# ideafisher/ssUnet-GAN

Hardware: AMD Instinct MI355X
Metric: train images/sec (512^2 tiles) (higher is better)
Workload: dtype f32; 1 GPU; UNet_R_SS_v2 generator + SRGAN-style discriminator, one G+D step (train_seg_gan.py:182-233), 16 x 3x512x512 tiles per GPU, fp32, Adam lr 2e-5; global_batch=16, tile=512, parallelism=dp1, dead_d_param_grads_of_g_step=computed

## Files before the change

### ssunet-gan_amd/csrc/conv_wgrad.hip

```cpp
#include "common.h"
#include "conv_thin.h"
#include "conv_wgrad_args.h"
#include <stdlib.h>

namespace {

constexpr int BKP = 16;

template <int BM, int BN, int WAVES_M, int WAVES_N>
__global__ __launch_bounds__(256) void wgrad_kernel(const WgArgs a) {
  constexpr int WTM = BM / WAVES_M, WTN = BN / WAVES_N;
  constexpr int MI = WTM / 32, NI = WTN / 32;
  constexpr int LDA = BM + 4, LDB = BN + 4;
  constexpr int AQ = BM / 4, BQ = BN / 4;
  constexpr int A_LD = BKP * AQ / 256, B_LD = (BKP * BQ + 255) / 256;
  constexpr int A_PSTEP = 256 / AQ, B_PSTEP = 256 / BQ;
  static_assert(A_LD >= 1, "tile");

  __shared__ __attribute__((aligned(16))) float lds[2 * BKP * (LDA + LDB)];
  float* As = lds;
  float* Bs = lds + 2 * BKP * LDA;

  const int tid = threadIdx.x, lane = tid & 63, wave = tid >> 6;
  const int wm = wave / WAVES_N, wn = wave % WAVES_N;
// ... 91 lines not shown
  }

  float* slab = a.ws + (size_t)blockIdx.z * a.M * a.Cout;
#pragma unroll
  for (int i = 0; i < MI; ++i)
#pragma unroll
    for (int j = 0; j < NI; ++j) {
      const int co = n0 + wn * WTN + j * 32 + l31;
#pragma unroll
      for (int r = 0; r < 16; ++r) {
        const int row = m0 + wm * WTM + i * 32 + (r & 3) + 8 * (r >> 2) + 4 * half;
        if (row < a.M && co < a.Cout) slab[(size_t)row * a.Cout + co] = acc[i][j][r];
      }
    }
}

struct RedArgs {
  const float* ws; float* dw; int splits, M, Cout, Cin, Cin_real, KH, KW, ntaps;
  int ky[SSG_MAX_TAPS], kx[SSG_MAX_TAPS];
};

template <int ZL>
__global__ __launch_bounds__(32 * ZL) void wgrad_reduce_kernel(const RedArgs a) {
  __shared__ float red[ZL][32];
  const int el = threadIdx.x & 31, zl = threadIdx.x >> 5;
  const long long idx = (long long)blockIdx.x * 32 + el;
  const long long tot = (long long)a.M * a.Cout;
  float s = 0.f;
  if (idx < tot) {
    int z = zl;
    for (; z + 3 * ZL < a.splits; z += 4 * ZL) {
      const float v0 = a.ws[(size_t)z * tot + idx], v1 = a.ws[(size_t)(z + ZL) * tot + idx];
      const float v2 = a.ws[(size_t)(z + 2 * ZL) * tot + idx], v3 = a.ws[(size_t)(z + 3 * ZL) * tot + idx];
      s += v0; s += v1; s += v2; s += v3;
    }
    for (; z < a.splits; z += ZL) s += a.ws[(size_t)z * tot + idx];
  }
  red[zl][el] = s;
  __syncthreads();
  if (zl != 0 || idx >= tot) return;
  float v = 0.f;
#pragma unroll
  for (int k = 0; k < ZL; ++k) v += red[k][el];
  const int row = (int)(idx / a.Cout), co = (int)(idx - (long long)row * a.Cout);
  const int t = row / a.Cin, c = row - t * a.Cin;
  if (c >= a.Cin_real) return;
  a.dw[(((size_t)co * a.Cin_real + c) * a.KH + a.ky[t]) * a.KW + a.kx[t]] = v;
}

struct Plan { int variant, mt, nt, splits, steps_per_split, halo; };

int wgrad4_kind(const ssg_wgrad_desc* d) {
  static const int on = [] { const char* e = getenv("SSG_WGRAD4"); return e ? atoi(e) : 1; }();
  return on ? ssg_wgrad4_kind(d) : 0;
}

bool wgrad_uses_dma(int variant) {
  static const int use_dma = [] { const char* e = getenv("SSG_WGRAD_DMA"); return e ? atoi(e) : 1; }();
  return use_dma && variant <= 1;
}

bool wgrad_uses_halo(const ssg_wgrad_desc* d, int variant) {
  static const int on = [] { const char* e = getenv("SSG_WGRAD_HALO"); return e ? atoi(e) : 1; }();
  return on && variant <= 1 && wgrad_uses_dma(variant) && ssg_wgrad_halo_ok(d, variant);
}

Plan make_plan(const ssg_wgrad_desc* d) {
  Plan p;
  p.halo = 0;
  const int Cin = d->C1 + d->C2;
  const int M = d->ntaps * Cin;
  int bn;
  if (d->Cout > 64) { p.variant = 0; bn = 128; }
  else if (d->Cout > 32) { p.variant = 1; bn = 64; }
  else { p.variant = 2; bn = 32; }
  p.mt = (M + 127) / 128;
  p.nt = (d->Cout + bn - 1) / bn;
  long long steps = ((long long)d->N * d->GH * d->GW + BKP - 1) / BKP;
  if (wgrad_uses_halo(d, p.variant)) {
    p.halo = 1;
    p.mt = Cin / ssg_wgrad_halo_cb(p.variant);
    steps = (long long)d->N * d->GH * ((d->GW + BKP - 1) / BKP);
  }
  if ((d->flags & 1) && ssg_wgrad_k32_ok(d)) {
    p.halo = 2;
    p.mt = Cin / 64; p.nt = d->Cout / 64;
    steps = ssg_wgrad_k32_steps(d);
    const long long tiles = (long long)p.mt * p.nt;
    long long max_rows = 128;
    {
      const long long steps16 = (long long)d->N * d->GH * ((d->GW + BKP - 1) / BKP);
      const long long mtf = Cin / ssg_wgrad_halo_cb(p.variant), ntf = (d->Cout + (p.variant == 0 ? 127 : 63)) / (p.variant == 0 ? 128 : 64);
      long long wantf = 1024 / (mtf * ntf > 0 ? mtf * ntf : 1);
      if (wantf < 1) wantf = 1;
      if (wantf > steps16 / 16) wantf = steps16 / 16 > 0 ? steps16 / 16 : 1;
      if (wantf > 512) wantf = 512;
      const long long chain_px = (steps16 + wantf - 1) / wantf * BKP;
      if (chain_px / 32 < max_rows) max_rows = chain_px / 32;
      if (max_rows < 8) max_rows = 8;
    }
    const long long lo = ssg_wgrad_k32_flush() == 0 ? (steps + max_rows - 1) / max_rows : 1;
    long long hi = steps / 8;
    if (hi < lo) hi = lo;
    long long best = lo; double beff = 0;
    for (long long sp = lo; sp <= hi && sp <= lo + 1024; ++sp) {
      const long long wg = sp * tiles;
      const double eff = (double)wg / (256.0 * ((wg + 255) / 256));
      if (eff > beff + 1e-9) { beff = eff; best = sp; }
      if (eff >= 0.97 && wg >= 256) break;
    }
    p.steps_per_split = (int)((steps + best - 1) / best);
    p.splits = (int)((steps + p.steps_per_split - 1) / p.steps_per_split);
    return p;
  }
  static const int wgs = [] { const char* e = getenv("SSG_WGRAD_WGS"); return e ? atoi(e) : 1024; }();
  long long want = wgs / ((long long)p.mt * p.nt);
  if (want < 1) want = 1;
  long long maxs = steps / 16;
  if (maxs < 1) maxs = 1;
  if (want > maxs) want = maxs;
  if (want > 512) want = 512;
  p.steps_per_split = (int)((steps + want - 1) / want);
  p.splits = (int)((steps + p.steps_per_split - 1) / p.steps_per_split);
  return p;
}

int validate(const ssg_wgrad_desc* d) {
  SSG_REQUIRE(d && d->in1 && d->dout && d->dw_oihw, SSG_EINVAL, "wgrad: null pointer");
  SSG_REQUIRE(d->C1 > 0 && d->C1 % 4 == 0 && d->C2 >= 0 && d->C2 % 4 == 0, SSG_EINVAL, "wgrad: channels must be multiples of 4");
  SSG_REQUIRE(d->C2 == 0 || d->in2, SSG_EINVAL, "wgrad: C2 > 0 needs in2");
  SSG_REQUIRE(d->ld1 % 4 == 0 && d->ld1 >= d->C1 && d->ldd % 4 == 0 && d->ldd >= d->Cout, SSG_EALIGN, "wgrad: strides");
  SSG_REQUIRE(d->C2 == 0 || (d->ld2 % 4 == 0 && d->ld2 >= d->C2), SSG_EALIGN, "wgrad: ld2");
  SSG_REQUIRE(ssg_aligned16(d->in1) && ssg_aligned16(d->in2) && ssg_aligned16(d->dout) && ssg_aligned16(d->ws), SSG_EALIGN, "wgrad: alignment");
  SSG_REQUIRE(d->ntaps >= 1 && d->ntaps <= SSG_MAX_TAPS, SSG_EINVAL, "wgrad: ntaps");
  SSG_REQUIRE(d->Cin_real > 0 && d->Cin_real <= d->C1 + d->C2, SSG_EINVAL, "wgrad: Cin_real");
  for (int t = 0; t < d->ntaps; ++t) {
    SSG_REQUIRE(d->dy[t] >= -2 && d->dy[t] <= 5 && d->dx[t] >= -2 && d->dx[t] <= 5, SSG_EINVAL, "wgrad: tap offset");
    SSG_REQUIRE(d->ky[t] >= 0 && d->ky[t] < d->KH && d->kx[t] >= 0 && d->kx[t] < d->KW, SSG_EINVAL, "wgrad: kernel position");
  }
  SSG_REQUIRE(d->ws_bytes >= ssg_conv2d_wgrad_workspace_bytes(d), SSG_EINVAL, "wgrad: workspace too small");
  return SSG_OK;
}

__global__ __launch_bounds__(256) void pack_weights_kernel(const float* __restrict__ w, int O, int I, int KH, int KW,
                                                           int transpose, int ntaps, unsigned long long kpos_bits,
                                                           int kmode, int Cred_pad, int Kp, int R, float* __restrict__ out,
                                                           const float* __restrict__ sigma) {
  const long long idx = (long long)blockIdx.x * 256 + threadIdx.x;
  if (idx >= (long long)R * Kp) return;
  const int r = (int)(idx / Kp), k = (int)(idx - (long long)r * Kp);
  int t, c;
  if (kmode == 0) {
    const int span = ntaps * 16;
    const int chunk = k / span, rem = k - chunk * span;
    t = rem >> 4; c = chunk * 16 + (rem & 15);
  } else {
    t = k / Cred_pad; c = k - t * Cred_pad;
  }
  const int Cred = transpose ? O : I;
  float v = 0.f;
  if (t < ntaps && c < Cred) {
    const int kb = (int)((kpos_bits >> (6 * t)) & 63ull);
    const int ky = kb & 7, kx = kb >> 3;
    const int o = transpose ? c : r, i = transpose ? r : c;
    v = w[(((size_t)o * I + i) * KH + ky) * KW + kx];
    if (sigma) v *= 1.f / *sigma;
  }
  out[idx] = v;
}

}

extern "C" int64_t ssg_conv2d_wgrad_workspace_bytes(const ssg_wgrad_desc* d) {
  if (!d) return 0;
  if (wgrad4_kind(d)) {
    const int nz = ssg_wgrad4_slices(d, wgrad4_kind(d), nullptr, nullptr, nullptr);
    return (int64_t)nz * d->ntaps * (d->C1 + d->C2) * d->Cout * (int64_t)sizeof(float);
  }
  const Plan p = make_plan(d);
  return (int64_t)p.splits * d->ntaps * (d->C1 + d->C2) * d->Cout * (int64_t)sizeof(float);
}

extern "C" int ssg_conv2d_wgrad_in_affine_ok(const ssg_wgrad_desc* d) {
  if (!d || !d->in1 || !d->dout || wgrad4_kind(d)) return 0;
  if (d->C2 != 0 || (d->in_act != SSG_ACT_NONE && d->in_act != SSG_ACT_RELU && d->in_act != SSG_ACT_LRELU)) return 0;
  return make_plan(d).halo == 2 ? 1 : 0;
}

extern "C" int ssg_conv2d_wgrad_f32(const ssg_wgrad_desc* d, void* stream) {
  int rc = validate(d);
  if (rc != SSG_OK) return rc;
  SSG_REQUIRE(!d->in_scale || (d->in_shift && ssg_conv2d_wgrad_in_affine_ok(d)), SSG_EINVAL,
              "wgrad: in_scale on a descriptor whose kernel has no fused input transform (ssg_conv2d_wgrad_in_affine_ok == 0)");
  Plan p = make_plan(d);
  hipStream_t st = (hipStream_t)stream;
  const int w4 = wgrad4_kind(d);
  WgArgs a;
  a.in1 = d->in1; a.in2 = d->C2 ? d->in2 : d->in1; a.dout = d->dout; a.ws = d->ws;
  a.C1 = d->C1; a.C2 = d->C2; a.ld1 = d->ld1; a.ld2 = d->C2 ? d->ld2 : d->ld1;
  a.N = d->N; a.H = d->H; a.W = d->W; a.Cout = d->Cout; a.ldd = d->ldd; a.GH = d->GH; a.GW = d->GW;
  a.in_sy = d->in_sy; a.in_sx = d->in_sx; a.ntaps = d->ntaps;
  a.tap_bits = 0;
  for (int t = 0; t < d->ntaps; ++t)
    a.tap_bits |= (unsigned long long)(((d->dy[t] + 2) & 7) | (((d->dx[t] + 2) & 7) << 3)) << (6 * t);
  a.in_scale = d->in_scale; a.in_shift = d->in_shift; a.in_act = d->in_act; a.in_slope = d->in_slope;
  a.M = d->ntaps * (d->C1 + d->C2);
  a.Ptot = (long long)d->N * d->GH * d->GW;
  a.steps_per_split = p.steps_per_split;
  if (w4) {
    p.splits = ssg_wgrad4_slices(d, w4, nullptr, nullptr, nullptr);
    rc = ssg_wgrad4_launch(d, w4, st);
    if (rc != SSG_OK) return rc;
  } else {
    dim3 grid((unsigned)p.mt, (unsigned)p.nt, (unsigned)p.splits);
    if (p.halo == 2) {
      rc = ssg_wgrad_k32_launch(a, grid, st);
      if (rc != SSG_OK) return rc;
    } else if (p.halo) {
      rc = ssg_wgrad_halo_launch(a, p.variant, grid, st, (d->flags & 1) != 0);
      if (rc != SSG_OK) return rc;
    } else if (wgrad_uses_dma(p.variant)) {
      rc = ssg_wgrad_dma_launch(a, p.variant, grid, st, (d->flags & 1) != 0);
      if (rc != SSG_OK) return rc;
    } else
    switch (p.variant) {
      case 0: hipLaunchKernelGGL((wgrad_kernel<128, 128, 2, 2>), grid, dim3(256), 0, st, a); break;
      case 1: hipLaunchKernelGGL((wgrad_kernel<128, 64, 2, 2>), grid, dim3(256), 0, st, a); break;
      default: hipLaunchKernelGGL((wgrad_kernel<128, 32, 4, 1>), grid, dim3(256), 0, st, a); break;
    }
    SSG_LAUNCH_CHECK();
  }
  RedArgs r;
  r.ws = d->ws; r.dw = d->dw_oihw; r.splits = p.splits; r.M = a.M; r.Cout = d->Cout; r.Cin = d->C1 + d->C2;
  r.Cin_real = d->Cin_real; r.KH = d->KH; r.KW = d->KW; r.ntaps = d->ntaps;
  for (int t = 0; t < SSG_MAX_TAPS; ++t) { r.ky[t] = t < d->ntaps ? d->ky[t] : 0; r.kx[t] = t < d->ntaps ? d->kx[t] : 0; }
  const long long tot = (long long)a.M * d->Cout;
  if (p.splits >= 256 && tot <= 32 * 1024)
    hipLaunchKernelGGL(wgrad_reduce_kernel<32>, dim3((unsigned)ssg_cdiv(tot, 32)), dim3(1024), 0, st, r);
  else
    hipLaunchKernelGGL(wgrad_reduce_kernel<8>, dim3((unsigned)ssg_cdiv(tot, 32)), dim3(256), 0, st, r);
  SSG_LAUNCH_CHECK();
  return SSG_OK;
}

extern "C" int ssg_pack_weights_scaled_f32(const float* w_oihw, int O, int I, int KH, int KW, int transpose, int ntaps,
                                           const int* ky, const int* kx, int kmode, int Cred_pad, int Kp, const float* sigma, float* out,
                                           void* stream);
extern "C" int ssg_pack_weights_f32(const float* w_oihw, int O, int I, int KH, int KW, int transpose, int ntaps,
                                    const int* ky, const int* kx, int kmode, int Cred_pad, int Kp, float* out,
                                    void* stream) {
  return ssg_pack_weights_scaled_f32(w_oihw, O, I, KH, KW, transpose, ntaps, ky, kx, kmode, Cred_pad, Kp, nullptr, out, stream);
}
extern "C" int ssg_pack_weights_scaled_f32(const float* w_oihw, int O, int I, int KH, int KW, int transpose, int ntaps,
                                           const int* ky, const int* kx, int kmode, int Cred_pad, int Kp, const float* sigma, float* out,
                                           void* stream) {
  SSG_REQUIRE(w_oihw && out && ky && kx, SSG_EINVAL, "pack: null pointer");
  SSG_REQUIRE(ntaps >= 1 && ntaps <= SSG_MAX_TAPS && KH <= 8 && KW <= 8, SSG_EINVAL, "pack: taps");
  SSG_REQUIRE(Kp % 16 == 0 && Cred_pad % 4 == 0, SSG_EINVAL, "pack: Kp/Cred_pad");
  const int Cred = transpose ? O : I;
  SSG_REQUIRE(Cred_pad >= Cred, SSG_EINVAL, "pack: Cred_pad < reduced channels");
  if (kmode == 0) SSG_REQUIRE(Cred_pad % 16 == 0 && Kp == ntaps * Cred_pad, SSG_EINVAL, "pack: kmode 0 shape");
  else SSG_REQUIRE(Kp >= ntaps * Cred_pad, SSG_EINVAL, "pack: kmode 1 Kp");
  unsigned long long bits = 0;
  for (int t = 0; t < ntaps; ++t) {
    SSG_REQUIRE(ky[t] >= 0 && ky[t] < KH && kx[t] >= 0 && kx[t] < KW, SSG_EINVAL, "pack: kernel position");
    bits |= (unsigned long long)(ky[t] | (kx[t] << 3)) << (6 * t);
  }
  const int R = transpose ? I : O;
  const long long tot = (long long)R * Kp;
  hipLaunchKernelGGL(pack_weights_kernel, dim3((unsigned)ssg_cdiv(tot, 256)), dim3(256), 0, (hipStream_t)stream,
                     w_oihw, O, I, KH, KW, transpose, ntaps, bits, kmode, Cred_pad, Kp, R, out, sigma);
  SSG_LAUNCH_CHECK();
  return SSG_OK;
}

extern "C" int ssg_conv2d_wgrad_kernel_id(const ssg_wgrad_desc* d) {
  if (!d) return SSG_EINVAL;
  if (wgrad4_kind(d)) return 10 + wgrad4_kind(d);
  if (make_plan(d).halo == 2) return 60;
  if (make_plan(d).halo) return ((d->flags & 1) ? 40 : 30) + make_plan(d).variant;
  const int v = make_plan(d).variant;
  return v + (wgrad_uses_dma(v) ? ((d->flags & 1) ? 50 : 20) : 0);
}
```

### ssunet-gan_amd/csrc/conv_wgrad_args.h

```cpp
#pragma once
#include "common.h"

struct WgArgs {
  const float* in1; const float* in2; const float* dout; float* ws;
  int C1, C2, ld1, ld2, N, H, W, Cout, ldd, GH, GW, in_sy, in_sx, ntaps;
  unsigned long long tap_bits;
  int M;
  long long Ptot;
  int steps_per_split;
  int xcd_swizzle;
  const float* in_scale; const float* in_shift; int in_act; float in_slope;
};


int ssg_wgrad_dma_launch(const WgArgs& a, int variant, dim3 grid, hipStream_t st, bool split);

int ssg_wgrad_halo_cb(int variant);
bool ssg_wgrad_halo_ok(const ssg_wgrad_desc* d, int variant);
int ssg_wgrad_halo_launch(const WgArgs& a, int variant, dim3 grid, hipStream_t st, bool split);

bool ssg_wgrad_k32_ok(const ssg_wgrad_desc* d);
long long ssg_wgrad_k32_steps(const ssg_wgrad_desc* d);
int ssg_wgrad_k32_flush();
int ssg_wgrad_k32_launch(const WgArgs& a, dim3 grid, hipStream_t st);
```

### ssunet-gan_amd/csrc/conv_wgrad_k32.hip

```cpp
#include "common.h"
#include "lds_dma.h"
#include "conv_wgrad_args.h"
#include "mfma_split.h"
#include "conv_slow.h"
#include <stdlib.h>

namespace {

typedef unsigned u32x4 __attribute__((ext_vector_type(4)));
typedef short s16x4 __attribute__((ext_vector_type(4)));
typedef short s16x8 __attribute__((ext_vector_type(8)));
typedef __attribute__((address_space(3))) s16x4 lds_s16x4;

constexpr int KP = 32;
constexpr int WPX = 36;
constexpr int XSLOT = WPX * 128;
constexpr int XPLANE = 4 * XSLOT;
constexpr int XIMG = 3 * XPLANE;
constexpr int DSLOT = KP * 128;
constexpr int DPLANE = 2 * DSLOT;
constexpr int DIMG = 3 * DPLANE;
constexpr int CB = 64, BN = 64;
#ifndef SSG_WK32_FLUSH
#define SSG_WK32_FLUSH 0
#endif

__device__ __forceinline__ int sw(int p) { return ((((p >> 1) & 1) | (((p >> 3) & 1) << 1)) << 1); }

template <bool XF>
__global__ __launch_bounds__(512, 1) void wgrad_k32_kernel(const WgArgs a) {
  extern __shared__ __attribute__((aligned(1024))) unsigned char lds[];
  unsigned char* const ximg = lds;
  unsigned char* const dimg = lds + XIMG;

  const int tid = threadIdx.x, lane = tid & 63;
  const int wave = __builtin_amdgcn_readfirstlane(tid >> 6);
  const int wm = wave >> 1, wn = wave & 1;
  const int l15 = lane & 15, g = lane >> 4;
  const int c0 = blockIdx.x * CB, n0 = blockIdx.y * BN;
  const int Cin = a.C1 + a.C2;
  const int XB = (a.GW + KP - 1) / KP;

  const long long total = (long long)a.N * XB * a.GH;
  long long S0 = (long long)blockIdx.z * a.steps_per_split, S1 = S0 + a.steps_per_split;
  if (S1 > total) S1 = total;

  const unsigned OOB = 0xffffffffu;
  const bool first = c0 < a.C1;
  const float* xsrc = first ? a.in1 : a.in2;
  const int xld = first ? a.ld1 : a.ld2;
  const int xc0 = first ? c0 : c0 - a.C1;
  const unsigned npix = (unsigned)a.N * (unsigned)a.H * (unsigned)a.W;
  const auto x_rs = __builtin_amdgcn_make_buffer_rsrc(const_cast<float*>(xsrc), 0, (int)(npix * (unsigned)xld * 4u), 0x00020000);
  const auto d_rs = __builtin_amdgcn_make_buffer_rsrc(const_cast<float*>(a.dout), 0, (int)((unsigned)a.N * (unsigned)a.GH * (unsigned)a.GW * (unsigned)a.ldd * 4u), 0x00020000);

  const int s_px = tid >> 4, s_q = tid & 15;
  const bool has_x2 = tid < 32;
  const int x_dst = s_px * 128 + (((s_q >> 1) ^ sw(s_px)) << 4) + (s_q & 1) * 8;
  const int x_dst2 = (32 + s_px) * 128 + (((s_q >> 1) ^ sw(32 + s_px)) << 4) + (s_q & 1) * 8;
  const int d_dst = x_dst;

  struct RawX { u32x4 a, b; };
  struct RawD { u32x4 a; };
  float* const xtab = (float*)(lds + XIMG + DIMG);
  if constexpr (XF) {
    if (tid < 128) xtab[tid] = tid < 64 ? a.in_scale[c0 + tid] : a.in_shift[c0 + tid - 64];
  }
  auto x_inside = [&](int row, int gx0, int px) -> bool {
    return (unsigned)row < (unsigned)a.H && (unsigned)(gx0 - 1 + px) < (unsigned)a.W;
  };
  auto load_x = [&](int n, int row, int gx0) -> RawX {
    const unsigned rowbase = (unsigned)((n * a.H + row) * a.W + gx0 - 1);
    const unsigned cho = (unsigned)(xc0 + 4 * s_q) * 4u;
    const unsigned vo = x_inside(row, gx0, s_px) ? (rowbase + (unsigned)s_px) * (unsigned)xld * 4u + cho : OOB;
    const unsigned vo2 = (has_x2 && x_inside(row, gx0, 32 + s_px)) ? (rowbase + 32u + (unsigned)s_px) * (unsigned)xld * 4u + cho : OOB;
    RawX r;
    r.a = __builtin_amdgcn_raw_buffer_load_b128(x_rs, vo, 0, 0);
    r.b = __builtin_amdgcn_raw_buffer_load_b128(x_rs, vo2, 0, 0);
    return r;
  };
  auto load_d = [&](int n, int gy, int gx0) -> RawD {
    const int gx = gx0 + s_px;
    const unsigned vo = gx < a.GW ? (unsigned)((n * a.GH + gy) * a.GW + gx) * (unsigned)a.ldd * 4u + (unsigned)(n0 + 4 * s_q) * 4u : OOB;
    RawD r;
    r.a = __builtin_amdgcn_raw_buffer_load_b128(d_rs, vo, 0, 0);
    return r;
  };
  auto put = [&](unsigned char* base, int plane_bytes, f32x4 v) {
    bf16x4 p1, p2, p3;
    split3_4(v, p1, p2, p3);
    *(bf16x4*)base = p1; *(bf16x4*)(base + plane_bytes) = p2; *(bf16x4*)(base + 2 * plane_bytes) = p3;
  };
  auto xform = [&](f32x4 v, bool inside) -> f32x4 {
    if constexpr (XF) {
      v = v * *(const f32x4*)(xtab + 4 * s_q) + *(const f32x4*)(xtab + 64 + 4 * s_q);
#pragma unroll
      for (int e = 0; e < 4; ++e) v[e] = ssg_act(v[e], a.in_act, a.in_slope);
      if (!inside) v = f32x4{0.f, 0.f, 0.f, 0.f};
    }
    return v;
  };
  auto store_x = [&](const RawX& r, int slot, int row, int gx0) {
    put(ximg + slot * XSLOT + x_dst, XPLANE, xform(__builtin_bit_cast(f32x4, r.a), XF ? x_inside(row, gx0, s_px) : true));
    if (has_x2) put(ximg + slot * XSLOT + x_dst2, XPLANE, xform(__builtin_bit_cast(f32x4, r.b), XF ? x_inside(row, gx0, 32 + s_px) : true));
  };
  auto store_d = [&](const RawD& r, int slot) {
    put(dimg + slot * DSLOT + d_dst, DPLANE, __builtin_bit_cast(f32x4, r.a));
  };

  const int q4 = l15 >> 2, pp = l15 & 3;
  int xoff[3][2], doff[2][2];
#pragma unroll
  for (int t = 0; t < 2; ++t) {
#pragma unroll
    for (int dx = 0; dx < 3; ++dx) {
      const int p = dx + 8 * g + q4 + 4 * t;
      xoff[dx][t] = p * 128 + ((((2 * wm + (pp >> 1)) ^ sw(p))) << 4) + (pp & 1) * 8;
    }
    const int p = 8 * g + q4 + 4 * t;
#pragma unroll
    for (int j = 0; j < 2; ++j)
      doff[j][t] = p * 128 + ((((2 * (2 * wn + j) + (pp >> 1)) ^ sw(p))) << 4) + (pp & 1) * 8;
  }

  constexpr int FLUSH = SSG_WK32_FLUSH;
  f32x4 acc[9][2], tot[9][2];
#pragma unroll
  for (int t = 0; t < 9; ++t)
#pragma unroll
    for (int j = 0; j < 2; ++j) { acc[t][j] = f32x4{0.f, 0.f, 0.f, 0.f}; tot[t][j] = f32x4{0.f, 0.f, 0.f, 0.f}; }
  int since = 0;

  auto frag = [&](const unsigned char* base, int o0, int o1) -> bf16x8 {
    const s16x4 lo = __builtin_amdgcn_ds_read_tr16_b64_v4i16((lds_s16x4*)(base + o0));
    const s16x4 hi = __builtin_amdgcn_ds_read_tr16_b64_v4i16((lds_s16x4*)(base + o1));
    const s16x8 v = __builtin_shufflevector(lo, hi, 0, 1, 2, 3, 4, 5, 6, 7);
    return __builtin_bit_cast(bf16x8, v);
  };

  long long S = S0;
  while (S < S1) {
    const int strip = (int)(S / a.GH), ga = (int)(S - (long long)strip * a.GH);
    long long Se = (long long)(strip + 1) * a.GH;
    if (Se > S1) Se = S1;
    const int gb = ga + (int)(Se - S);
    const int n = strip / XB, gx0 = (strip - n * XB) * KP;

    wait_lds_reads();
    __builtin_amdgcn_s_barrier();
    asm volatile("" ::: "memory");
    {
      const RawX r0 = load_x(n, ga - 1, gx0), r1 = load_x(n, ga, gx0), r2 = load_x(n, ga + 1, gx0);
      const RawD r3 = load_d(n, ga, gx0);
      store_x(r0, (ga + 0) & 3, ga - 1, gx0); store_x(r1, (ga + 1) & 3, ga, gx0);
      store_x(r2, (ga + 2) & 3, ga + 1, gx0); store_d(r3, ga & 1);
    }

    for (int gy = ga; gy < gb; ++gy) {
      wait_lds_reads();
      __builtin_amdgcn_s_barrier();
      asm volatile("" ::: "memory");
      const bool more = gy + 1 < gb;
      RawX nx; RawD nd;
#ifndef SSG_WK32_LOAD_MID
#define SSG_WK32_LOAD_MID 0
#endif
#if !SSG_WK32_LOAD_MID
      if (more) { nx = load_x(n, gy + 2, gx0); nd = load_d(n, gy + 1, gx0); }
#endif

      const unsigned char* db = dimg + (gy & 1) * DSLOT;
      bf16x8 df[2][3];
#pragma unroll
      for (int j = 0; j < 2; ++j)
#pragma unroll
        for (int q = 0; q < 3; ++q) df[j][q] = frag(db + q * DPLANE, doff[j][0], doff[j][1]);
#pragma unroll
      for (int dyi = 0; dyi < 3; ++dyi) {
#ifndef SSG_WK32_DYNPRIO
#define SSG_WK32_DYNPRIO 1
#endif
        if (SSG_WK32_DYNPRIO) { if (dyi == 0) __builtin_amdgcn_s_setprio(3); else if (dyi == 1) __builtin_amdgcn_s_setprio(2); else __builtin_amdgcn_s_setprio(1); }
        const unsigned char* xb = ximg + ((gy + dyi) & 3) * XSLOT;
        bf16x8 xf[3][3];
#pragma unroll
        for (int dx = 0; dx < 3; ++dx)
#pragma unroll
          for (int q = 0; q < 3; ++q) xf[dx][q] = frag(xb + q * XPLANE, xoff[dx][0], xoff[dx][1]);
#define SSG_WK_TERM(QD, QX)                                                                       \
  _Pragma("unroll") for (int dx = 0; dx < 3; ++dx)                                                \
  _Pragma("unroll") for (int j = 0; j < 2; ++j)                                                   \
      acc[dyi * 3 + dx][j] = __builtin_amdgcn_mfma_f32_16x16x32_bf16(df[j][QD], xf[dx][QX], acc[dyi * 3 + dx][j], 0, 0, 0);
        SSG_WK_TERM(2, 0) SSG_WK_TERM(1, 1) SSG_WK_TERM(0, 2)
        SSG_WK_TERM(1, 0) SSG_WK_TERM(0, 1)
        SSG_WK_TERM(0, 0)
#undef SSG_WK_TERM
#if SSG_WK32_LOAD_MID
        if (dyi == 0) {
          __builtin_amdgcn_sched_barrier(0);
          if (more) { nx = load_x(n, gy + 2, gx0); nd = load_d(n, gy + 1, gx0); }
          __builtin_amdgcn_sched_barrier(0);
        }
#endif
      }
      if (SSG_WK32_DYNPRIO) __builtin_amdgcn_s_setprio(0);
      if (more) {
        __builtin_amdgcn_sched_barrier(0);
        store_x(nx, (gy + 3) & 3, gy + 2, gx0);
        store_d(nd, (gy + 1) & 1);
      }
      if (FLUSH > 0 && ++since == FLUSH) {
        since = 0;
#pragma unroll
        for (int t = 0; t < 9; ++t)
#pragma unroll
          for (int j = 0; j < 2; ++j) { tot[t][j] += acc[t][j]; acc[t][j] = f32x4{0.f, 0.f, 0.f, 0.f}; }
      }
    }
    S = Se;
  }
#pragma unroll
  for (int t = 0; t < 9; ++t)
#pragma unroll
    for (int j = 0; j < 2; ++j) tot[t][j] += acc[t][j];

  wait_lds_reads();
  {
    bool bad = false;
#pragma unroll
    for (int t = 0; t < 9; ++t)
#pragma unroll
      for (int j = 0; j < 2; ++j)
#pragma unroll
        for (int r = 0; r < 4; ++r) bad |= ssg_nonfinite(tot[t][j][r]);
    if (__builtin_amdgcn_readfirstlane(__syncthreads_or(bad))) {
      const WgArgs& as = *ssg_reload_args<WgArgs>();
#pragma unroll
      for (int t = 0; t < 9; ++t)
#pragma unroll
        for (int j = 0; j < 2; ++j)
          ssg_slow_refill4(tot[t][j], (float*)lds + tid, 512, [&](int r) {
            return ssg_wgrad_slow_value_strips<XF>(as, t, c0 + wm * 16 + l15, n0 + (2 * wn + j) * 16 + 4 * g + r, S0, S1, KP);
          });
    }
  }

  float* slab = a.ws + (size_t)blockIdx.z * a.M * a.Cout;
  const int ci = c0 + wm * 16 + l15;
#pragma unroll
  for (int t = 0; t < 9; ++t)
#pragma unroll
    for (int j = 0; j < 2; ++j)
      *(f32x4*)(slab + ((size_t)t * Cin + ci) * a.Cout + n0 + (2 * wn + j) * 16 + 4 * g) = tot[t][j];
}

}

static int g_wk32_mode = -1;
extern "C" int ssg_wgrad_set_k32_mode(int mode) {
  SSG_REQUIRE(mode == 0 || mode == 1, SSG_EINVAL, "wgrad k32 mode %d", mode);
  g_wk32_mode = mode;
  return SSG_OK;
}

bool ssg_wgrad_k32_ok(const ssg_wgrad_desc* d) {
  if (g_wk32_mode < 0) { const char* e = getenv("SSG_WGRAD_K32"); g_wk32_mode = e ? atoi(e) : 1; }
  if (!g_wk32_mode || !(d->flags & 1)) return false;
  if (d->ntaps != 9 || d->in_sy != 1 || d->in_sx != 1 || d->GH != d->H || d->GW != d->W) return false;
  for (int t = 0; t < 9; ++t)
    if (d->dy[t] != t / 3 - 1 || d->dx[t] != t % 3 - 1) return false;
  if (d->C1 % 64 || d->C2 % 64 || d->Cout % 64 || d->GW < 17) return false;
  if ((d->ld1 & 3) || (d->C2 && (d->ld2 & 3)) || (d->ldd & 3)) return false;
  const unsigned long long xb = (unsigned long long)d->N * d->H * d->W * (unsigned long long)(d->ld1 > d->ld2 ? d->ld1 : d->ld2) * 4ull;
  const unsigned long long db = (unsigned long long)d->N * d->GH * d->GW * (unsigned long long)d->ldd * 4ull;
  return xb <= 0xfffffff0ull && db <= 0xfffffff0ull;
}

int ssg_wgrad_k32_flush() { return SSG_WK32_FLUSH; }

long long ssg_wgrad_k32_steps(const ssg_wgrad_desc* d) { return (long long)d->N * ((d->GW + KP - 1) / KP) * d->GH; }

int ssg_wgrad_k32_launch(const WgArgs& a, dim3 grid, hipStream_t st) {
  constexpr int lds_bytes = XIMG + DIMG;
  static const hipError_t attr = hipFuncSetAttribute((const void*)wgrad_k32_kernel<false>, hipFuncAttributeMaxDynamicSharedMemorySize, lds_bytes);
  static const hipError_t attr_xf = hipFuncSetAttribute((const void*)wgrad_k32_kernel<true>, hipFuncAttributeMaxDynamicSharedMemorySize, lds_bytes + 512);
  if (attr != hipSuccess || attr_xf != hipSuccess) { ssg_set_error("wgrad k32: LDS attribute: %s", hipGetErrorString(attr != hipSuccess ? attr : attr_xf)); return (int)(attr != hipSuccess ? attr : attr_xf); }
  if (a.in_scale) hipLaunchKernelGGL(wgrad_k32_kernel<true>, grid, dim3(512), lds_bytes + 512, st, a);
  else hipLaunchKernelGGL(wgrad_k32_kernel<false>, grid, dim3(512), lds_bytes, st, a);
  SSG_LAUNCH_CHECK();
  return SSG_OK;
}
```

### ssunet-gan_amd/ops.py

```python
import ctypes as C
import math

import torch
import torch.distributed as dist

from . import _lib
from ._lib import ACT_LRELU, ACT_NONE, ACT_RELU, ConvDesc, WgradDesc, call, ptr, stream_ptr

__all__ = ['conv2d', 'batch_norm_act', 'max_pool2x2', 'max_pool2x2_skip', 'max_unpool2x2', 'upsample2x_bilinear', 'upsample2x_nearest',
           'spade_modulate', 'adaptive_avgpool_flat', 'linear', 'seg_loss', 'bce_with_logits_const', 'nan_to_zero_',
           'to_nhwc', 'new_nhwc', 'bump_weight_epoch', 'dwconv2d', 'swish', 'sigmoid', 'gaussian', 'mul', 'global_avgpool',
           'channel_scale', 'spectral_norm_weight', 'conv2d_sn']


def pad4(c):
    return (c + 3) // 4 * 4


def new_nhwc(n, c, h, w, device, ld=None, zero=False):
    ld = pad4(c) if ld is None else ld
    buf = (torch.zeros if zero else torch.empty)(n * h * w * ld, device=device, dtype=torch.float32)
    return torch.empty(0, device=device, dtype=torch.float32).set_(
        buf.untyped_storage(), 0, (n, c, h, w), (h * w * ld, 1, w * ld, ld))

# ... 99 lines not shown
    cache = weight.__dict__.get('_ssg_pack')
    if cache is None or cache[0] != stamp:
        cache = (stamp, {})
        try:
            weight._ssg_pack = cache
        except Exception:
            pass
    key = (transpose, tuple(taps), cred_pad, kmode)
    hit = cache[1].get(key)
    if hit is not None:
        return hit, kp, kmode
    out = torch.empty((rows, kp), device=weight.device, dtype=torch.float32)
    ky = (C.c_int * nt)(*[t[0] for t in taps])
    kx = (C.c_int * nt)(*[t[1] for t in taps])
    call('ssg_pack_weights_f32', ptr(weight), o, i, kh, kw, int(transpose), nt, ky, kx, kmode, cred_pad, kp, ptr(out), stream_ptr())
    cache[1][key] = out
    return out, kp, kmode


def _fill_taps(desc, taps):
    desc.ntaps = len(taps)
    for t, (_, _, dy, dx) in enumerate(taps):
        desc.dy[t] = dy
        desc.dx[t] = dx


PROFILE = None
PROFILE_SHAPES = False
PROFILE_HBM = None
PROFILE_COMM = None
_ROLE = [None]


def _timed_all_reduce(kind, t, group):
    if PROFILE_COMM is None:
        dist.all_reduce(t, op=dist.ReduceOp.SUM, group=group)
        return
    e0 = torch.cuda.Event(enable_timing=True); e1 = torch.cuda.Event(enable_timing=True)
    e0.record(torch.cuda.current_stream())
    dist.all_reduce(t, op=dist.ReduceOp.SUM, group=group)
    e1.record(torch.cuda.current_stream())
    PROFILE_COMM.append((kind, t.numel() * t.element_size(), e0, e1))


class role(object):

    def __init__(self, name):
        self.name = name

    def __enter__(self):
        self.prev = _ROLE[0]; _ROLE[0] = self.name

    def __exit__(self, *a):
        _ROLE[0] = self.prev


class _hbm(object):

    def __init__(self, stage, nbytes):
        self.rec = PROFILE_HBM is not None
        if self.rec:
            self.stage, self.nbytes = stage, float(nbytes)
            self.e0 = torch.cuda.Event(enable_timing=True); self.e1 = torch.cuda.Event(enable_timing=True)

    def __enter__(self):
        if self.rec:
            self.e0.record(torch.cuda.current_stream())

    def __exit__(self, *a):
        if self.rec:
            self.e1.record(torch.cuda.current_stream())
            PROFILE_HBM.append((self.stage, self.nbytes, self.e0, self.e1))


_CONV_LABELS = {0: 'conv_igemm_kernel<128,128>', 1: 'conv_igemm_kernel<256,64>', 2: 'conv_igemm_kernel<256,32>',
                20: 'conv_igemm_dma_kernel<128,128>', 21: 'conv_igemm_dma_kernel<256,64>', 22: 'conv_igemm_dma_kernel<128,64>',
                30: 'conv_igemm_halo_kernel<128,128>', 31: 'conv_igemm_halo_kernel<256,64>', 32: 'conv_igemm_halo_kernel<128,64>',
                33: 'conv_igemm_halo16_kernel<128,128>', 34: 'conv_igemm_halo16_kernel<128,64>',
                10: 'thin_small_cout_kernel',
                12: 'thin4_cin_kernel', 13: 'thin4_cout_kernel', 14: 'tiny4_kernel', 15: 'thin32_cin_kernel', 16: 'conv1x1_k64_kernel'}
_WGRAD_LABELS = {0: 'wgrad_kernel<128,128>', 1: 'wgrad_kernel<128,64>', 2: 'wgrad_kernel<128,32>',
                 20: 'wgrad_dma_kernel<128,128>', 21: 'wgrad_dma_kernel<128,64>',
                 30: 'wgrad_halo_kernel<32,128>', 31: 'wgrad_halo_kernel<64,64>',
                 40: 'wgrad_halo_x3_kernel<32,128>', 41: 'wgrad_halo_x3_kernel<64,64>', 60: 'wgrad_k32_kernel<64,64>',
                 50: 'wgrad_dma_x3_kernel<128,128>', 51: 'wgrad_dma_x3_kernel<128,64>',
                 15: 'wgrad4_kernel<thin_cout>', 16: 'wgrad4_kernel<thin_cin>', 17: 'wgrad_tiny4_kernel', 18: 'wgrad32_cin_kernel'}


class _Timed(object):
    def __init__(self, label, flops, tag=None):
        self.rec = PROFILE is not None
        if self.rec:
            self.label, self.flops, self.tag = label, flops, tag
            self.e0 = torch.cuda.Event(enable_timing=True); self.e1 = torch.cuda.Event(enable_timing=True)

    def __enter__(self):
        if self.rec:
            self.e0.record(torch.cuda.current_stream())

    def __exit__(self, *a):
        if self.rec:
            self.e1.record(torch.cuda.current_stream())
            PROFILE.append((self.label, self.flops, self.e0, self.e1, self.tag))


_DECLINED = object()


def _conv_launch(x1, x2, wpk, kp, kmode, row0, cout, bias, res, act, slope, taps, n, h, w, gh, gw, oh, ow,
                 in_s, out_s, out_oy, out_ox, out, want_bn=False, tag=None, parity_merge=False, in_affine=None, bwd_stats=None):
    d = ConvDesc()
    d.in1 = x1.data_ptr(); d.C1 = pad4(x1.shape[1]); d.ld1 = _ld(x1)
    if x2 is not None:
        d.in2 = x2.data_ptr(); d.C2 = pad4(x2.shape[1]); d.ld2 = _ld(x2)
    else:
        d.in2 = None; d.C2 = 0; d.ld2 = 0
    d.N, d.H, d.W = n, h, w
    d.w = wpk.data_ptr() + row0 * kp * 4; d.Kp = kp; d.kmode = kmode
    d.bias = bias.data_ptr() if bias is not None else None
    if res is not None:
        d.res = res.data_ptr(); d.ldr = _ld(res)
    else:
        d.res = None; d.ldr = 0
    d.out = out.data_ptr(); d.Cout = cout; d.ldo = _ld(out)
    d.GH, d.GW, d.OH, d.OW = gh, gw, oh, ow
    d.in_sy = d.in_sx = in_s
    d.out_sy = d.out_sx = out_s
    d.out_oy, d.out_ox = out_oy, out_ox
    _fill_taps(d, taps)
    d.act = act; d.slope = slope
    d.bnpart = None
    d.ws = None; d.ws_bytes = 0
    d.w_split = None
    d.parity_merge = 1 if parity_merge else 0
    d.in_scale = None; d.in_shift = None; d.in_act = ACT_NONE; d.in_slope = 0.0
    d.bwd_x = None; d.bwd_ldx = 0; d.bwd_scale = None; d.bwd_shift = None; d.bwd_mean = None; d.bwd_act = ACT_NONE; d.bwd_slope = 0.0
    split = None
    if parity_merge and not (MFMA_SPLIT and kmode == 0 and call('ssg_conv2d_split_bn', C.byref(d)) == 64):
        return False
    if MFMA_SPLIT and kmode == 0:
        bn = call('ssg_conv2d_split_bn', C.byref(d))
        if bn:
            split = _split_pack(wpk, row0, cout, kp, 1064 if bn == 2064 else bn)
            d.w_split = split.data_ptr()
    if in_affine is not None:
        d.in_scale = in_affine[0].data_ptr(); d.in_shift = in_affine[1].data_ptr(); d.in_act = int(in_affine[2]); d.in_slope = float(in_affine[3])
        if split is None or not call('ssg_conv2d_in_affine_ok', C.byref(d)):
            return _DECLINED
        bn = call('ssg_conv2d_split_bn', C.byref(d))
    if bwd_stats is not None:
        bx, bst, bact, bslope = bwd_stats
        d.bwd_x = bx.data_ptr(); d.bwd_ldx = _ld(bx); d.bwd_scale = bst[2].data_ptr(); d.bwd_shift = bst[3].data_ptr()
        d.bwd_mean = bst[0].data_ptr(); d.bwd_act = int(bact); d.bwd_slope = float(bslope)
        if split is None or not call('ssg_conv2d_bwd_stats_ok', C.byref(d)):
            return _DECLINED
        want_bn = True
    part = None
    if want_bn and BN_EPILOGUE:
        rows = call('ssg_conv2d_bnpart_rows', C.byref(d))
        if rows > 0:
            part = torch.empty((rows, 2, cout), dtype=torch.float64, device=out.device)
            d.bnpart = part.data_ptr()
    if bwd_stats is not None and part is None:
        return _DECLINED
    ws = None
    if part is None and split is None:
        need = call('ssg_conv2d_workspace_bytes', C.byref(d))
# ... 1210 lines not shown
```

Baseline: 85.63 images/sec.

## Extend k32 weight-gradient kernel to stride-2 3x3 convolutions

Adds a stride-2 variant of the LDS-staged k32 wgrad kernel. Input rows are stored de-interleaved by even and odd column in a five-slot ring, and two input rows are loaded per output row. This routes stride-2 3x3 convs, which previously fell back to the generic or DMA wgrad kernels, onto the faster fused path. The path is gated on having enough tiles to fill the GPU, and it needs more LDS and an extra row load per step.

```diff
diff --git a/ssunet-gan_amd/csrc/conv_wgrad.hip b/ssunet-gan_amd/csrc/conv_wgrad.hip
--- a/ssunet-gan_amd/csrc/conv_wgrad.hip
+++ b/ssunet-gan_amd/csrc/conv_wgrad.hip
@@ -197,13 +197,23 @@
     p.mt = Cin / ssg_wgrad_halo_cb(p.variant);
     steps = (long long)d->N * d->GH * ((d->GW + BKP - 1) / BKP);
   }
-  if ((d->flags & 1) && ssg_wgrad_k32_ok(d)) {
-    p.halo = 2;
+  const bool k32_s2 = (d->flags & 1) && !p.halo && ssg_wgrad_k32_s2_ok(d);
+  if (((d->flags & 1) && ssg_wgrad_k32_ok(d)) || k32_s2) {
+    p.halo = k32_s2 ? 3 : 2;
     p.mt = Cin / 64; p.nt = d->Cout / 64;
     steps = ssg_wgrad_k32_steps(d);
     const long long tiles = (long long)p.mt * p.nt;
     long long max_rows = 128;
-    {
+    if (k32_s2) {
+      const long long steps16 = ((long long)d->N * d->GH * d->GW + BKP - 1) / BKP;
+      long long wantf = 1024 / ((long long)((M + 127) / 128) * ((d->Cout + bn - 1) / bn));
+      if (wantf < 1) wantf = 1;
+      if (wantf > steps16 / 16) wantf = steps16 / 16 > 0 ? steps16 / 16 : 1;
+      if (wantf > 512) wantf = 512;
+      const long long chain_px = (steps16 + wantf - 1) / wantf * BKP;
+      if (chain_px / 32 < max_rows) max_rows = chain_px / 32;
+      if (max_rows < 8) max_rows = 8;
+    } else {
       const long long steps16 = (long long)d->N * d->GH * ((d->GW + BKP - 1) / BKP);
       const long long mtf = Cin / ssg_wgrad_halo_cb(p.variant), ntf = (d->Cout + (p.variant == 0 ? 127 : 63)) / (p.variant == 0 ? 128 : 64);
       long long wantf = 1024 / (mtf * ntf > 0 ? mtf * ntf : 1);
@@ -328,7 +338,7 @@
     if (rc != SSG_OK) return rc;
   } else {
     dim3 grid((unsigned)p.mt, (unsigned)p.nt, (unsigned)p.splits);
-    if (p.halo == 2) {
+    if (p.halo >= 2) {
       rc = ssg_wgrad_k32_launch(a, grid, st);
       if (rc != SSG_OK) return rc;
     } else if (p.halo) {
@@ -393,6 +403,7 @@
   if (!d) return SSG_EINVAL;
   if (wgrad4_kind(d)) return 10 + wgrad4_kind(d);
   if (make_plan(d).halo == 2) return 60;
+  if (make_plan(d).halo == 3) return 61;
   if (make_plan(d).halo) return ((d->flags & 1) ? 40 : 30) + make_plan(d).variant;
   const int v = make_plan(d).variant;
   return v + (wgrad_uses_dma(v) ? ((d->flags & 1) ? 50 : 20) : 0);
diff --git a/ssunet-gan_amd/csrc/conv_wgrad_args.h b/ssunet-gan_amd/csrc/conv_wgrad_args.h
--- a/ssunet-gan_amd/csrc/conv_wgrad_args.h
+++ b/ssunet-gan_amd/csrc/conv_wgrad_args.h
@@ -20,6 +20,7 @@
 int ssg_wgrad_halo_launch(const WgArgs& a, int variant, dim3 grid, hipStream_t st, bool split);
 
 bool ssg_wgrad_k32_ok(const ssg_wgrad_desc* d);
+bool ssg_wgrad_k32_s2_ok(const ssg_wgrad_desc* d);
 long long ssg_wgrad_k32_steps(const ssg_wgrad_desc* d);
 int ssg_wgrad_k32_flush();
 int ssg_wgrad_k32_launch(const WgArgs& a, dim3 grid, hipStream_t st);
diff --git a/ssunet-gan_amd/csrc/conv_wgrad_k32.hip b/ssunet-gan_amd/csrc/conv_wgrad_k32.hip
--- a/ssunet-gan_amd/csrc/conv_wgrad_k32.hip
+++ b/ssunet-gan_amd/csrc/conv_wgrad_k32.hip
@@ -13,10 +13,13 @@
 typedef __attribute__((address_space(3))) s16x4 lds_s16x4;
 
 constexpr int KP = 32;
-constexpr int WPX = 36;
-constexpr int XSLOT = WPX * 128;
-constexpr int XPLANE = 4 * XSLOT;
-constexpr int XIMG = 3 * XPLANE;
+template <bool S2> struct XGeo {
+  static constexpr int WPX = S2 ? 65 : 36, NSLOT = S2 ? 5 : 4;
+  static constexpr int XSLOT = WPX * 128;
+  static constexpr int XPLANE = NSLOT * XSLOT;
+  static constexpr int XIMG = 3 * XPLANE;
+};
+constexpr int S2_EVEN = 33;
 constexpr int DSLOT = KP * 128;
 constexpr int DPLANE = 2 * DSLOT;
 constexpr int DIMG = 3 * DPLANE;
@@ -27,8 +30,10 @@
 
 __device__ __forceinline__ int sw(int p) { return ((((p >> 1) & 1) | (((p >> 3) & 1) << 1)) << 1); }
 
-template <bool XF>
+template <bool XF, bool S2>
 __global__ __launch_bounds__(512, 1) void wgrad_k32_kernel(const WgArgs a) {
+  static_assert(!(XF && S2), "the stride-2 form has no fused input transform");
+  constexpr int XSLOT = XGeo<S2>::XSLOT, XPLANE = XGeo<S2>::XPLANE, XIMG = XGeo<S2>::XIMG;
   extern __shared__ __attribute__((aligned(1024))) unsigned char lds[];
   unsigned char* const ximg = lds;
   unsigned char* const dimg = lds + XIMG;
@@ -55,28 +60,36 @@
   const auto d_rs = __builtin_amdgcn_make_buffer_rsrc(const_cast<float*>(a.dout), 0, (int)((unsigned)a.N * (unsigned)a.GH * (unsigned)a.GW * (unsigned)a.ldd * 4u), 0x00020000);
 
   const int s_px = tid >> 4, s_q = tid & 15;
-  const bool has_x2 = tid < 32;
-  const int x_dst = s_px * 128 + (((s_q >> 1) ^ sw(s_px)) << 4) + (s_q & 1) * 8;
-  const int x_dst2 = (32 + s_px) * 128 + (((s_q >> 1) ^ sw(32 + s_px)) << 4) + (s_q & 1) * 8;
-  const int d_dst = x_dst;
-
-  struct RawX { u32x4 a, b; };
+  const bool has_x2 = S2 || tid < 32, has_x3 = S2 && tid < 16;
+  auto piece = [&](int row) { return row * 128 + (((s_q >> 1) ^ sw(row)) << 4) + (s_q & 1) * 8; };
+  auto xrow = [&](int w) { return S2 ? ((w & 1) ? S2_EVEN + (w >> 1) : w >> 1) : w; };
+  const int x_dst = piece(xrow(s_px));
+  const int x_dst2 = piece(xrow(32 + s_px));
+  const int x_dst3 = piece(xrow(64));
+  const int d_dst = piece(s_px);
+  auto xslot = [&](int row) { return S2 ? (row + 1) % 5 : (row + 1) & 3; };
+
+  struct RawX { u32x4 a, b, c; };
   struct RawD { u32x4 a; };
   float* const xtab = (float*)(lds + XIMG + DIMG);
   if constexpr (XF) {
     if (tid < 128) xtab[tid] = tid < 64 ? a.in_scale[c0 + tid] : a.in_shift[c0 + tid - 64];
   }
-  auto x_inside = [&](int row, int gx0, int px) -> bool {
-    return (unsigned)row < (unsigned)a.H && (unsigned)(gx0 - 1 + px) < (unsigned)a.W;
-  };
-  auto load_x = [&](int n, int row, int gx0) -> RawX {
-    const unsigned rowbase = (unsigned)((n * a.H + row) * a.W + gx0 - 1);
+  auto x_inside = [&](int row, int wx0, int px) -> bool {
+    return (unsigned)row < (unsigned)a.H && (unsigned)(wx0 + px) < (unsigned)a.W;
+  };
+  auto load_x = [&](int n, int row, int wx0) -> RawX {
+    const unsigned rowbase = (unsigned)((n * a.H + row) * a.W + wx0);
     const unsigned cho = (unsigned)(xc0 + 4 * s_q) * 4u;
-    const unsigned vo = x_inside(row, gx0, s_px) ? (rowbase + (unsigned)s_px) * (unsigned)xld * 4u + cho : OOB;
-    const unsigned vo2 = (has_x2 && x_inside(row, gx0, 32 + s_px)) ? (rowbase + 32u + (unsigned)s_px) * (unsigned)xld * 4u + cho : OOB;
+    const unsigned vo = x_inside(row, wx0, s_px) ? (rowbase + (unsigned)s_px) * (unsigned)xld * 4u + cho : OOB;
+    const unsigned vo2 = (has_x2 && x_inside(row, wx0, 32 + s_px)) ? (rowbase + 32u + (unsigned)s_px) * (unsigned)xld * 4u + cho : OOB;
     RawX r;
     r.a = __builtin_amdgcn_raw_buffer_load_b128(x_rs, vo, 0, 0);
     r.b = __builtin_amdgcn_raw_buffer_load_b128(x_rs, vo2, 0, 0);
+    if constexpr (S2) {
+      const unsigned vo3 = (has_x3 && x_inside(row, wx0, 64)) ? (rowbase + 64u) * (unsigned)xld * 4u + cho : OOB;
+      r.c = __builtin_amdgcn_raw_buffer_load_b128(x_rs, vo3, 0, 0);
+    }
     return r;
   };
   auto load_d = [&](int n, int gy, int gx0) -> RawD {
@@ -100,9 +113,11 @@
     }
     return v;
   };
-  auto store_x = [&](const RawX& r, int slot, int row, int gx0) {
-    put(ximg + slot * XSLOT + x_dst, XPLANE, xform(__builtin_bit_cast(f32x4, r.a), XF ? x_inside(row, gx0, s_px) : true));
-    if (has_x2) put(ximg + slot * XSLOT + x_dst2, XPLANE, xform(__builtin_bit_cast(f32x4, r.b), XF ? x_inside(row, gx0, 32 + s_px) : true));
+  auto store_x = [&](const RawX& r, int row, int wx0) {
+    const int slot = xslot(row);
+    put(ximg + slot * XSLOT + x_dst, XPLANE, xform(__builtin_bit_cast(f32x4, r.a), XF ? x_inside(row, wx0, s_px) : true));
+    if (has_x2) put(ximg + slot * XSLOT + x_dst2, XPLANE, xform(__builtin_bit_cast(f32x4, r.b), XF ? x_inside(row, wx0, 32 + s_px) : true));
+    if (has_x3) put(ximg + slot * XSLOT + x_dst3, XPLANE, __builtin_bit_cast(f32x4, r.c));
   };
   auto store_d = [&](const RawD& r, int slot) {
     put(dimg + slot * DSLOT + d_dst, DPLANE, __builtin_bit_cast(f32x4, r.a));
@@ -114,7 +129,8 @@
   for (int t = 0; t < 2; ++t) {
 #pragma unroll
     for (int dx = 0; dx < 3; ++dx) {
-      const int p = dx + 8 * g + q4 + 4 * t;
+      const int i = 8 * g + q4 + 4 * t;
+      const int p = S2 ? (dx == 1 ? S2_EVEN + i : i + (dx >> 1)) : dx + i;
       xoff[dx][t] = p * 128 + ((((2 * wm + (pp >> 1)) ^ sw(p))) << 4) + (pp & 1) * 8;
     }
     const int p = 8 * g + q4 + 4 * t;
@@ -145,15 +161,17 @@
     if (Se > S1) Se = S1;
     const int gb = ga + (int)(Se - S);
     const int n = strip / XB, gx0 = (strip - n * XB) * KP;
+    const int wx0 = S2 ? 2 * gx0 - 1 : gx0 - 1;
+    const int ya = S2 ? 2 * ga : ga;
 
     wait_lds_reads();
     __builtin_amdgcn_s_barrier();
     asm volatile("" ::: "memory");
     {
-      const RawX r0 = load_x(n, ga - 1, gx0), r1 = load_x(n, ga, gx0), r2 = load_x(n, ga + 1, gx0);
+      const RawX r0 = load_x(n, ya - 1, wx0), r1 = load_x(n, ya, wx0), r2 = load_x(n, ya + 1, wx0);
       const RawD r3 = load_d(n, ga, gx0);
-      store_x(r0, (ga + 0) & 3, ga - 1, gx0); store_x(r1, (ga + 1) & 3, ga, gx0);
-      store_x(r2, (ga + 2) & 3, ga + 1, gx0); store_d(r3, ga & 1);
+      store_x(r0, ya - 1, wx0); store_x(r1, ya, wx0);
+      store_x(r2, ya + 1, wx0); store_d(r3, ga & 1);
     }
 
     for (int gy = ga; gy < gb; ++gy) {
@@ -161,12 +179,13 @@
       __builtin_amdgcn_s_barrier();
       asm volatile("" ::: "memory");
       const bool more = gy + 1 < gb;
-      RawX nx; RawD nd;
+      const int y = S2 ? 2 * gy : gy;
+      RawX nx, nx2; RawD nd;
 #ifndef SSG_WK32_LOAD_MID
 #define SSG_WK32_LOAD_MID 0
 #endif
 #if !SSG_WK32_LOAD_MID
-      if (more) { nx = load_x(n, gy + 2, gx0); nd = load_d(n, gy + 1, gx0); }
+      if (more) { nx = load_x(n, y + 2, wx0); if (S2) nx2 = load_x(n, y + 3, wx0); nd = load_d(n, gy + 1, gx0); }
 #endif
 
       const unsigned char* db = dimg + (gy & 1) * DSLOT;
@@ -181,7 +200,7 @@
 #define SSG_WK32_DYNPRIO 1
 #endif
         if (SSG_WK32_DYNPRIO) { if (dyi == 0) __builtin_amdgcn_s_setprio(3); else if (dyi == 1) __builtin_amdgcn_s_setprio(2); else __builtin_amdgcn_s_setprio(1); }
-        const unsigned char* xb = ximg + ((gy + dyi) & 3) * XSLOT;
+        const unsigned char* xb = ximg + xslot(y - 1 + dyi) * XSLOT;
         bf16x8 xf[3][3];
 #pragma unroll
         for (int dx = 0; dx < 3; ++dx)
@@ -198,7 +217,7 @@
 #if SSG_WK32_LOAD_MID
         if (dyi == 0) {
           __builtin_amdgcn_sched_barrier(0);
-          if (more) { nx = load_x(n, gy + 2, gx0); nd = load_d(n, gy + 1, gx0); }
+          if (more) { nx = load_x(n, y + 2, wx0); if (S2) nx2 = load_x(n, y + 3, wx0); nd = load_d(n, gy + 1, gx0); }
           __builtin_amdgcn_sched_barrier(0);
         }
 #endif
@@ -206,7 +225,8 @@
       if (SSG_WK32_DYNPRIO) __builtin_amdgcn_s_setprio(0);
       if (more) {
         __builtin_amdgcn_sched_barrier(0);
-        store_x(nx, (gy + 3) & 3, gy + 2, gx0);
+        store_x(nx, y + 2, wx0);
+        if (S2) store_x(nx2, y + 3, wx0);
         store_d(nd, (gy + 1) & 1);
       }
       if (FLUSH > 0 && ++since == FLUSH) {
@@ -258,15 +278,18 @@
 
 static int g_wk32_mode = -1;
 extern "C" int ssg_wgrad_set_k32_mode(int mode) {
-  SSG_REQUIRE(mode == 0 || mode == 1, SSG_EINVAL, "wgrad k32 mode %d", mode);
+  SSG_REQUIRE(mode >= 0 && mode <= 2, SSG_EINVAL, "wgrad k32 mode %d", mode);
   g_wk32_mode = mode;
   return SSG_OK;
 }
 
-bool ssg_wgrad_k32_ok(const ssg_wgrad_desc* d) {
+static int wk32_mode() {
   if (g_wk32_mode < 0) { const char* e = getenv("SSG_WGRAD_K32"); g_wk32_mode = e ? atoi(e) : 1; }
-  if (!g_wk32_mode || !(d->flags & 1)) return false;
-  if (d->ntaps != 9 || d->in_sy != 1 || d->in_sx != 1 || d->GH != d->H || d->GW != d->W) return false;
+  return g_wk32_mode;
+}
+
+static bool k32_common_ok(const ssg_wgrad_desc* d) {
+  if (d->ntaps != 9) return false;
   for (int t = 0; t < 9; ++t)
     if (d->dy[t] != t / 3 - 1 || d->dx[t] != t % 3 - 1) return false;
   if (d->C1 % 64 || d->C2 % 64 || d->Cout % 64 || d->GW < 17) return false;
@@ -276,17 +299,39 @@
   return xb <= 0xfffffff0ull && db <= 0xfffffff0ull;
 }
 
+bool ssg_wgrad_k32_ok(const ssg_wgrad_desc* d) {
+  if (!wk32_mode() || !(d->flags & 1)) return false;
+  if (d->in_sy != 1 || d->in_sx != 1 || d->GH != d->H || d->GW != d->W) return false;
+  return k32_common_ok(d);
+}
+
+long long ssg_wgrad_k32_steps(const ssg_wgrad_desc* d) { return (long long)d->N * ((d->GW + KP - 1) / KP) * d->GH; }
+
+bool ssg_wgrad_k32_s2_ok(const ssg_wgrad_desc* d) {
+  const int mode = wk32_mode();
+  if (!mode || !(d->flags & 1) || d->in_scale) return false;
+  if (d->in_sy != 2 || d->in_sx != 2 || d->GH != (d->H - 1) / 2 + 1 || d->GW != (d->W - 1) / 2 + 1) return false;
+  if (!k32_common_ok(d)) return false;
+  if (mode == 2) return true;
+  const long long tiles = (long long)((d->C1 + d->C2) / 64) * (d->Cout / 64);
+  return tiles * ((ssg_wgrad_k32_steps(d) + 127) / 128) >= 256;
+}
+
 int ssg_wgrad_k32_flush() { return SSG_WK32_FLUSH; }
 
-long long ssg_wgrad_k32_steps(const ssg_wgrad_desc* d) { return (long long)d->N * ((d->GW + KP - 1) / KP) * d->GH; }
-
 int ssg_wgrad_k32_launch(const WgArgs& a, dim3 grid, hipStream_t st) {
-  constexpr int lds_bytes = XIMG + DIMG;
-  static const hipError_t attr = hipFuncSetAttribute((const void*)wgrad_k32_kernel<false>, hipFuncAttributeMaxDynamicSharedMemorySize, lds_bytes);
-  static const hipError_t attr_xf = hipFuncSetAttribute((const void*)wgrad_k32_kernel<true>, hipFuncAttributeMaxDynamicSharedMemorySize, lds_bytes + 512);
-  if (attr != hipSuccess || attr_xf != hipSuccess) { ssg_set_error("wgrad k32: LDS attribute: %s", hipGetErrorString(attr != hipSuccess ? attr : attr_xf)); return (int)(attr != hipSuccess ? attr : attr_xf); }
-  if (a.in_scale) hipLaunchKernelGGL(wgrad_k32_kernel<true>, grid, dim3(512), lds_bytes + 512, st, a);
-  else hipLaunchKernelGGL(wgrad_k32_kernel<false>, grid, dim3(512), lds_bytes, st, a);
+  constexpr int lds_bytes = XGeo<false>::XIMG + DIMG, lds_s2 = XGeo<true>::XIMG + DIMG;
+  static_assert(lds_s2 <= 160 * 1024, "LDS");
+  static const hipError_t attr = hipFuncSetAttribute((const void*)wgrad_k32_kernel<false, false>, hipFuncAttributeMaxDynamicSharedMemorySize, lds_bytes);
+  static const hipError_t attr_xf = hipFuncSetAttribute((const void*)wgrad_k32_kernel<true, false>, hipFuncAttributeMaxDynamicSharedMemorySize, lds_bytes + 512);
+  static const hipError_t attr_s2 = hipFuncSetAttribute((const void*)wgrad_k32_kernel<false, true>, hipFuncAttributeMaxDynamicSharedMemorySize, lds_s2);
+  const hipError_t bad = attr != hipSuccess ? attr : attr_xf != hipSuccess ? attr_xf : attr_s2;
+  if (bad != hipSuccess) { ssg_set_error("wgrad k32: LDS attribute: %s", hipGetErrorString(bad)); return (int)bad; }
+  if (a.in_sy == 2) {
+    SSG_REQUIRE(!a.in_scale, SSG_EINVAL, "wgrad k32: the stride-2 form has no fused input transform");
+    hipLaunchKernelGGL((wgrad_k32_kernel<false, true>), grid, dim3(512), lds_s2, st, a);
+  } else if (a.in_scale) hipLaunchKernelGGL((wgrad_k32_kernel<true, false>), grid, dim3(512), lds_bytes + 512, st, a);
+  else hipLaunchKernelGGL((wgrad_k32_kernel<false, false>), grid, dim3(512), lds_bytes, st, a);
   SSG_LAUNCH_CHECK();
   return SSG_OK;
 }
diff --git a/ssunet-gan_amd/ops.py b/ssunet-gan_amd/ops.py
--- a/ssunet-gan_amd/ops.py
+++ b/ssunet-gan_amd/ops.py
@@ -205,7 +205,7 @@
 _WGRAD_LABELS = {0: 'wgrad_kernel<128,128>', 1: 'wgrad_kernel<128,64>', 2: 'wgrad_kernel<128,32>',
                  20: 'wgrad_dma_kernel<128,128>', 21: 'wgrad_dma_kernel<128,64>',
                  30: 'wgrad_halo_kernel<32,128>', 31: 'wgrad_halo_kernel<64,64>',
-                 40: 'wgrad_halo_x3_kernel<32,128>', 41: 'wgrad_halo_x3_kernel<64,64>', 60: 'wgrad_k32_kernel<64,64>',
+                 40: 'wgrad_halo_x3_kernel<32,128>', 41: 'wgrad_halo_x3_kernel<64,64>', 60: 'wgrad_k32_kernel<64,64>', 61: 'wgrad_k32_s2_kernel<64,64>',
                  50: 'wgrad_dma_x3_kernel<128,128>', 51: 'wgrad_dma_x3_kernel<128,64>',
                  15: 'wgrad4_kernel<thin_cout>', 16: 'wgrad4_kernel<thin_cin>', 17: 'wgrad_tiny4_kernel', 18: 'wgrad32_cin_kernel'}
 
```

After: 86.52 images/sec (median of 6 runs). 1.0% higher.
